# ruc-aimc-lab/LAFF

Hardware: AMD Instinct MI355X
Metric: text-video cosine pairs/sec (higher is better)
Workload: dtype f32 towers (FC on fp16 hi/lo split x3 MFMA) + fp16 similarity

## Files before the change

### laff_amd/csrc/api.hip

```cpp
#include <hip/hip_runtime.h>

#include <algorithm>
#include <climits>
#include <cmath>
#include <cstdarg>
#include <cstdio>
#include <cstdlib>
#include <cstring>
#include <string>
#include <vector>

#include "kernels.h"

constexpr int METRIC_SLOTS = 33;

struct laff_ctx {
    int device;
    hipStream_t stream;
    double* d_metrics = nullptr;
    unsigned metrics_slot = 0;
    double* h_metrics = nullptr;
    char* d_mscratch = nullptr;
};

// ... 1703 lines not shown
    *route = laff::gemm_route(a, sim_gemm_mode(precision), sim_gemm_aligned(K, precision));
    return LAFF_OK;
}

static int rank_prepare_impl(laff_ctx* ctx, const char* who, int sides, int emit, const float* Et, const float* Ev, const void* T,
                             const void* V, int Nt, int Nv, int H, int d, int precision, float prescale, const int* gt_col, int col0,
                             double* s_gt64, float* band_t, float* band_v, int* zero_count, unsigned* pairs) {
    if (int rc = bad_precision(who, precision)) return rc;
    if (Nt < 0 || Nv < 0 || H < 1 || d < 4 || (d & 3)) return fail(LAFF_E_SHAPE, "%s: need H >= 1, d %% 4 == 0 (Nt=%d Nv=%d H=%d d=%d)", who, Nt, Nv, H, d);
    if (!(prescale > 0.0f)) return fail(LAFF_E_ARG, "%s: prescale must be positive", who);
    if ((Et && !aligned16(Et)) || (Ev && !aligned16(Ev)) || (T && !aligned16(T)) || (V && !aligned16(V)))
        return fail(LAFF_E_ALIGN, "%s: embeddings and operands must be 16-byte aligned", who);
    DeviceGuard g(ctx->device);
    HIP_TRY(laff::launch_rank_prepare(Et, Ev, T, V, Nt, Nv, H, d, precision, prescale, gt_col, col0, s_gt64, band_t, band_v, zero_count,
                                      pairs, sides, ctx->stream, emit));
    return LAFF_OK;
}

int laff_rank_prepare(laff_ctx* ctx, const float* Et, const float* Ev, const void* T, const void* V, int Nt, int Nv, int H, int d,
                      int precision, float prescale, const int* gt_col, int col0, double* s_gt64, float* band_t, float* band_v,
                      int* zero_count, unsigned* pairs) {
    CHECK_CTX(ctx);
    if (Nt == 0 && Nv == 0) return LAFF_OK;
    if ((Nt > 0 && (!Et || !T || !gt_col || !s_gt64 || !band_t)) || (Nv > 0 && (!Ev || !V || !band_v)))
        return fail(LAFF_E_ARG, "laff_rank_prepare: null argument");
    return rank_prepare_impl(ctx, "laff_rank_prepare", 3, 0, Et, Ev, T, V, Nt, Nv, H, d, precision, prescale, gt_col, col0, s_gt64, band_t,
                             band_v, zero_count, pairs);
}

int laff_rank_prepare_part(laff_ctx* ctx, int sides, const float* Et, const float* Ev, const void* T, const void* V, int Nt, int Nv, int H,
                           int d, int precision, float prescale, const int* gt_col, int col0, double* s_gt64, float* band_t, float* band_v,
                           int* zero_count, unsigned* pairs) {
    CHECK_CTX(ctx);
    if (sides != 1 && sides != 2) return fail(LAFF_E_ARG, "laff_rank_prepare_part: sides must be 1 (text rows) or 2 (video rows)");
    if ((sides == 1 && Nt == 0) || (sides == 2 && Nv == 0)) return LAFF_OK;
    if (sides == 1 && (!Et || !T || !gt_col || !s_gt64 || !band_t || (Nv > 0 && !Ev))) return fail(LAFF_E_ARG, "laff_rank_prepare_part: null argument (text side)");
    if (sides == 2 && (!Ev || !V || !band_v)) return fail(LAFF_E_ARG, "laff_rank_prepare_part: null argument (video side)");
    return rank_prepare_impl(ctx, "laff_rank_prepare_part", sides, 0, Et, Ev, T, V, Nt, Nv, H, d, precision, prescale, gt_col, col0, s_gt64,
                             band_t, band_v, zero_count, pairs);
}

int laff_rank_prepare_emit(laff_ctx* ctx, int emit, const float* Et, const float* Ev, void* T, void* V, int Nt, int Nv, int H, int d,
                           int precision, float prescale, const int* gt_col, int col0, double* s_gt64, float* band_t, float* band_v,
                           int* zero_count, unsigned* pairs) {
    CHECK_CTX(ctx);
    if (emit < 1 || emit > 3) return fail(LAFF_E_ARG, "laff_rank_prepare_emit: emit must be 1 (T), 2 (V) or 3 (both)");
    if (precision != LAFF_PREC_FP16 && precision != LAFF_PREC_BF16)
        return fail(LAFF_E_UNSUPPORTED, "laff_rank_prepare_emit: single-plane 16-bit operands only (precision %d): call laff_pack_rows + laff_rank_prepare", precision);
    if (Nt == 0 || Nv == 0) return LAFF_OK;
    if (!Et || !Ev || !T || !V || !gt_col || !s_gt64 || !band_t || !band_v) return fail(LAFF_E_ARG, "laff_rank_prepare_emit: null argument");
    return rank_prepare_impl(ctx, "laff_rank_prepare_emit", 3, emit, Et, Ev, T, V, Nt, Nv, H, d, precision, prescale, gt_col, col0, s_gt64,
                             band_t, band_v, zero_count, pairs);
}

int laff_rank_export_pairs(laff_ctx* ctx, const double* s_gt64, int* count, float* S, int lds, int Nv, unsigned* pairs, unsigned pair_cap,
                           const int* bounds, int world, int col0, unsigned* out, unsigned cap, unsigned* fill) {
    CHECK_CTX(ctx);
    if (!s_gt64 || !count || !pairs || !bounds || !out || !fill) return fail(LAFF_E_ARG, "laff_rank_export_pairs: null argument");
    pair_cap &= ~3u;
    if (world < 1 || world > 16 || cap < 4 || (cap & 3) || pair_cap < 4) return fail(LAFF_E_SHAPE, "laff_rank_export_pairs: need 1 <= world <= 16, cap %% 4 == 0 (world=%d cap=%u)", world, cap);
    if (S && lds < Nv) return fail(LAFF_E_SHAPE, "laff_rank_export_pairs: lds=%d < Nv=%d", lds, Nv);
    if (!aligned16(out)) return fail(LAFF_E_ALIGN, "laff_rank_export_pairs: out must be 16-byte aligned");
    DeviceGuard g(ctx->device);
    HIP_TRY(laff::launch_rank_export(s_gt64, count, S, lds, pairs, pair_cap, bounds, world, col0, out, cap, fill, ctx->stream));
    return LAFF_OK;
}

static int rank_resolve_checks(const char* who, const float* Et, const float* Ev, int Nt, int Nv, int H, int d, const double* s_gt64,
                               const int* count, const float* S, int lds, const unsigned* pairs, unsigned& pair_cap) {
    if (!Et || !Ev || !s_gt64 || !count || !pairs) return fail(LAFF_E_ARG, "%s: null argument", who);
    pair_cap &= ~3u;
    if (Nt < 0 || Nv < 0 || H < 1 || d < 4 || (d & 3) || pair_cap < 4) return fail(LAFF_E_SHAPE, "%s: bad shape", who);
    if (S && lds < Nv) return fail(LAFF_E_SHAPE, "%s: lds=%d < Nv=%d", who, lds, Nv);
    if (!aligned16(Et) || !aligned16(Ev)) return fail(LAFF_E_ALIGN, "%s: embeddings must be 16-byte aligned", who);
    return LAFF_OK;
}

int laff_rank_resolve(laff_ctx* ctx, const float* Et, const float* Ev, int Nt, int Nv, int H, int d, const double* s_gt64,
                      int* count, float* S, int lds, unsigned* pairs, unsigned pair_cap) {
    CHECK_CTX(ctx);
    if (Nt == 0 || Nv == 0) return LAFF_OK;
    if (int rc = rank_resolve_checks("laff_rank_resolve", Et, Ev, Nt, Nv, H, d, s_gt64, count, S, lds, pairs, pair_cap)) return rc;
    DeviceGuard g(ctx->device);
    HIP_TRY(laff::launch_rank_resolve(Et, Ev, Nt, Nv, H, d, s_gt64, count, S, lds, pairs, pair_cap, ctx->stream));
    return LAFF_OK;
}

int laff_rank_resolve_metrics(laff_ctx* ctx, const float* Et, const float* Ev, int Nt, int Nv, int H, int d, const double* s_gt64,
                              int* count, float* S, int lds, unsigned* pairs, unsigned pair_cap, int base, int* ranks_out, double* out8,
                              int synchronous) {
    CHECK_CTX(ctx);
    if (!out8) return fail(LAFF_E_ARG, "laff_rank_resolve_metrics: null out8");
    if (Nt < 1 || Nv < 1) return fail(LAFF_E_SHAPE, "laff_rank_resolve_metrics: Nt=%d Nv=%d (the metrics of an empty query set are undefined)", Nt, Nv);
    if (int rc = rank_resolve_checks("laff_rank_resolve_metrics", Et, Ev, Nt, Nv, H, d, s_gt64, count, S, lds, pairs, pair_cap)) return rc;
    DeviceGuard g(ctx->device);
    if (int rc = metrics_buffers(ctx)) return rc;
    const size_t si = synchronous ? 0 : next_metrics_slot(ctx);
    double* slot = ctx->d_metrics + 8 * si;
    unsigned* ticket = (unsigned*)(ctx->d_mscratch + si * laff::rank_metrics_scratch_bytes() + laff::rank_resolve_ticket_offset());
    double* host8 = synchronous ? nullptr : pinned_alias(out8);
    HIP_TRY(laff::launch_rank_resolve(Et, Ev, Nt, Nv, H, d, s_gt64, count, S, lds, pairs, pair_cap, ctx->stream, Nt, base, ranks_out, slot,
                                      host8, ticket));
    if (synchronous) {
        if (int rc = metrics_read_back(ctx, out8, "laff_rank_resolve_metrics: a rank < 1 was found (the pair list of laff_sim_gemm_banded "
                                                  "overflowed, or the counts are corrupt)"))
            return rc;
        out8[7] = 0.0;
        return LAFF_OK;
    }
    if (!host8) HIP_TRY(hipMemcpyAsync(out8, slot, 8 * sizeof(double), hipMemcpyDeviceToHost, ctx->stream));
    return LAFF_OK;
}

int laff_gather_gt(laff_ctx* ctx, const float* S, int Nt, int Nv, int lds, const int* gt_col, int col0, float* s_gt) {
    CHECK_CTX(ctx);
    if (Nt == 0) return LAFF_OK;
    if (!S || !gt_col || !s_gt) return fail(LAFF_E_ARG, "laff_gather_gt: null argument");
    if (Nt < 0 || Nv < 0 || lds < Nv) return fail(LAFF_E_SHAPE, "laff_gather_gt: bad shape");
    DeviceGuard g(ctx->device);
    HIP_TRY(laff::launch_gather_gt(S, Nt, Nv, lds, gt_col, col0, s_gt, ctx->stream));
    return LAFF_OK;
}

int laff_rank_count(laff_ctx* ctx, const float* S, int Nt, int Nv, int lds, const int* gt_col, int col0,
                    const float* s_gt, int* count, int accumulate) {
    CHECK_CTX(ctx);
    if (Nt == 0) return LAFF_OK;
    if (!S || !gt_col || !s_gt || !count) return fail(LAFF_E_ARG, "laff_rank_count: null argument");
    if (Nt < 0 || Nv < 0 || lds < Nv) return fail(LAFF_E_SHAPE, "laff_rank_count: bad shape");
    DeviceGuard g(ctx->device);
    HIP_TRY(laff::launch_rank_count(S, Nt, Nv, lds, gt_col, col0, s_gt, count, accumulate, ctx->stream));
    return LAFF_OK;
}

int laff_topk_rows(laff_ctx* ctx, const float* S, int Nt, int Nv, int lds, int K, int* idx_out, float* val_out) {
    CHECK_CTX(ctx);
    if (Nt == 0) return LAFF_OK;
    if (!S || !idx_out || !val_out) return fail(LAFF_E_ARG, "laff_topk_rows: null argument");
    if (Nt < 0 || Nv < 1 || lds < Nv || K < 1 || K > Nv || K > 8192) return fail(LAFF_E_SHAPE, "laff_topk_rows: need 1 <= K <= min(Nv, 8192) (Nt=%d Nv=%d K=%d)", Nt, Nv, K);
    {
        const size_t kp = K <= 64 ? 64 : (K <= 512 ? 512 : (K <= 2048 ? 2048 : (K <= 4096 ? 4096 : 8192)));
        if ((size_t)((Nv + 3) & ~3) * 4 + kp * 8 + 256 * 4 + 16 > 160 * 1024)
            return fail(LAFF_E_UNSUPPORTED, "laff_topk_rows: Nv=%d with K=%d does not fit the LDS-resident row (%zu columns at most: split the "
                        "columns and merge the per-block lists, as laff_amd.ops.topk_rows does)", Nv, K, (160 * 1024 - kp * 8 - 1040) / 4);
    }
    DeviceGuard g(ctx->device);
    HIP_TRY(laff::launch_topk_rows(S, Nt, Nv, lds, K, idx_out, val_out, ctx->stream));
    return LAFF_OK;
}

int laff_v2t_count(laff_ctx* ctx, const float* S, int Nt, int Nv, int lds, const int* grp_off, const int* grp_idx,
                   int max_group, int* count) {
    CHECK_CTX(ctx);
    if (Nt == 0 || Nv == 0) return LAFF_OK;
    if (!S || !grp_off || !grp_idx || !count) return fail(LAFF_E_ARG, "laff_v2t_count: null argument");
    if (Nt < 0 || Nv < 0 || lds < Nv || max_group < 0) return fail(LAFF_E_SHAPE, "laff_v2t_count: bad shape");
    if (Nt == 0 || Nv == 0 || max_group == 0) return LAFF_OK;
    DeviceGuard g(ctx->device);
    HIP_TRY(laff::launch_v2t_count(S, Nt, Nv, lds, grp_off, grp_idx, max_group, count, ctx->stream));
    return LAFF_OK;
}

int laff_v2t_count_exact(laff_ctx* ctx, const float* S, int Nt, int Nv, int lds, const int* grp_off, const int* grp_idx,
                         int max_group, const float* Et, const float* Ev, int H, int d, const double* s_gt64,
                         const float* band_t, const float* band_v, int* count, unsigned* list, unsigned list_cap) {
    CHECK_CTX(ctx);
    if (Nt == 0 || Nv == 0) return LAFF_OK;
    if (!S || !grp_off || !grp_idx || !count || !Et || !Ev || !s_gt64 || !band_t || !band_v || !list)
        return fail(LAFF_E_ARG, "laff_v2t_count_exact: null argument");
    if (Nt < 0 || Nv < 0 || lds < Nv || max_group < 0 || H < 1 || d < 4 || (d & 3))
        return fail(LAFF_E_SHAPE, "laff_v2t_count_exact: bad shape (Nt=%d Nv=%d lds=%d H=%d d=%d: d must be a multiple of 4)", Nt, Nv, lds, H, d);
    if (!aligned16(Et) || !aligned16(Ev)) return fail(LAFF_E_ALIGN, "laff_v2t_count_exact: embeddings must be 16-byte aligned");
    if (list_cap < 1) return fail(LAFF_E_SHAPE, "laff_v2t_count_exact: list_cap must be >= 1");
    DeviceGuard g(ctx->device);
    if (max_group == 0) {
        HIP_TRY(hipMemsetAsync(count, 0, (size_t)Nt * sizeof(int), ctx->stream));
        HIP_TRY(hipMemsetAsync(list, 0, 16, ctx->stream));
        return LAFF_OK;
    }
    HIP_TRY(laff::launch_v2t_count_exact(S, Nt, Nv, lds, grp_off, grp_idx, max_group, Et, Ev, H, d, s_gt64, band_t, band_v, count, list,
                                         list_cap, ctx->stream));
    return LAFF_OK;
}

int laff_row_dot_gt(laff_ctx* ctx, const void* T, const void* V, int Nt, int Nv, int K, float scale, int precision,
// ... 41 lines not shown
```

### laff_amd/csrc/kernels.h

```cpp
#pragma once
#include <hip/hip_runtime.h>
#include <stdint.h>

#include "../../include/laff_hip.h"

namespace laff {

template <typename K>
static inline hipError_t smem_attr_once(unsigned long long& done, K kernel, int smem) {
    int dev = 0;
    hipError_t e = hipGetDevice(&dev);
    if (e != hipSuccess) return e;
    const unsigned long long bit = 1ull << (dev & 63);
    if (__atomic_load_n(&done, __ATOMIC_ACQUIRE) & bit) return hipSuccess;
    if (smem > 64 * 1024) {
        e = hipFuncSetAttribute((const void*)kernel, hipFuncAttributeMaxDynamicSharedMemorySize, smem);
        if (e != hipSuccess) return e;
    }
    __atomic_fetch_or(&done, bit, __ATOMIC_ACQ_REL);
    return hipSuccess;
}

enum { GEMM_F32 = 0, GEMM_F16 = 1, GEMM_BF16 = 2 };

// ... 147 lines not shown
    const float* g_values[MAX_L];
    const float* g_wt[MAX_L];
    const float* g_bias[MAX_L];
    int g_ldwt[MAX_L], g_dk[MAX_L];
    int head_major;
    int L, N, H, d;
    int head_stride;
    const float* w;
    const float* b;
    const float* gw;
    unsigned flags;
    float* E;
    float* attn_w;
    void* E16;
    int e16_bf16;
    float e16_scale;
    int rp_side;
    const int* rp_gt;
    int rp_col0, rp_Nv;
    const float* rp_Ev;
    double* rp_sgt;
    float* rp_band;
    float* rp_band_v;
    int* rp_count;
    unsigned* rp_pairs;
    double* rp_part;
    unsigned* rp_ticket;
    float rp_unit, rp_cacc;
};
hipError_t launch_fuse(const FuseArgs& a, hipStream_t st);
hipError_t launch_plane_row_norms(const FuseArgs& a, float* out , hipStream_t st);

struct FrameArgs {
    const float* frames;
    const int* lens;
    int B, Fmax, d;
    const float* w;
    const float* b;
    const float* gw;
    unsigned flags;
    float* V;
    const float* mask;
    int ldm;
};
struct FrameGroup {
    int count;
    FrameArgs f[8];
};
hipError_t launch_frame_fuse(const FrameGroup& g, hipStream_t st);

hipError_t launch_split_rows_grouped(int count, const float* const* X, const int* N, const int* K, const int* ldx, void* const* out,
                                     float* const* rscale, hipStream_t st);
hipError_t launch_loss_normalize(const float* s, const float* im, int B, int H, int d, int dp, int Bp, float eps, float* XH,
                                 float* XHT, float* nrm, float* npr, hipStream_t st);
hipError_t launch_margin_reduce(const float* S, float* dS, float* dST, float* loss_h, float* loss, int B, int Bp, int H,
                                float margin, int max_violation, int use_s, int use_im, float g_s, float g_im, hipStream_t st);
hipError_t launch_loss_normalize_bwd(const float* XH, const float* G, const float* nrm, const float* npr, int B, int H, int d,
                                     int dp, float* d_s, float* d_im, hipStream_t st);
hipError_t launch_loss_sum_heads(const float* loss_h, int H, float* loss, hipStream_t st);
constexpr int DSL_STAT_ROWS = 10;
hipError_t launch_dsl_reduce(const float* S, float* ST, float* stat, float* dS, float* dST, float* loss_h, float* loss, int B, int Bp,
                             int H, float temp, hipStream_t st);
hipError_t launch_fc_gather(const int* indptr, const int* indices, const float* values, int N, int Dk, const float* Wt, int ldwt,
                            const float* bias, const float* bn_scale, const float* bn_shift, int D, int act, float* Y, int ldy,
                            hipStream_t st);
hipError_t launch_pack_rows(const float* E, int N, int H, int d, int lde, int normalize, float eps, float prescale,
                            int precision, void* out, hipStream_t st);

hipError_t launch_row_dot_gt(const void* T, const void* V, int Nt, int Nv, int K, int bf16, int x3, float scale,
                             const int* gt_col, int col0, float* s_gt, int* zero_count, hipStream_t st);
static inline void rank_band_constants(int precision, int H, int d, float* unit, float* c_acc) {
    const bool x3 = precision == LAFF_PREC_FP16X3 || precision == LAFF_PREC_BF16X3;
    const bool bf16 = precision == LAFF_PREC_BF16 || precision == LAFF_PREC_BF16X3;
    *unit = precision == LAFF_PREC_FP32 ? 5.9604645e-8f : (bf16 ? 3.90625e-3f : 4.8828125e-4f);
    *c_acc = (float)((double)H * d * (x3 ? 3.0 : 1.0) * 1.1920929e-7 + 9.5367432e-7 + (x3 ? 2.3841858e-7 : 0.0));
}
hipError_t launch_rank_prepare(const float* Et, const float* Ev, const void* T, const void* V, int Nt, int Nv, int H, int d,
                               int precision, float prescale, const int* gt_col, int col0, double* s_gt64, float* band_t,
                               float* band_v, int* zero_count, unsigned* pairs, int sides, hipStream_t st, int emit = 0);
hipError_t launch_rank_export(const double* s_gt64, int* count, float* S, int lds, unsigned* pairs, unsigned pair_cap, const int* bounds,
                              int world, int col0, unsigned* out, unsigned cap, unsigned* fill, hipStream_t st);
hipError_t launch_rank_resolve(const float* Et, const float* Ev, int Nt, int Nv, int H, int d, const double* s_gt64, int* count,
                               float* S, int lds, unsigned* pairs, unsigned pair_cap, hipStream_t st, int metrics_n = 0, int base = 0,
                               int* ranks_out = nullptr, double* out8 = nullptr, double* host8 = nullptr, unsigned* ticket = nullptr);
size_t rank_metrics_scratch_bytes();
size_t rank_resolve_ticket_offset();
hipError_t launch_rank_metrics(const int* r, int n, int base, int* ranks_out, double* out7, double* err, unsigned* scratch, hipStream_t st,
                               double* host8 = nullptr);
hipError_t launch_gather_gt(const float* S, int Nt, int Nv, int lds, const int* gt_col, int col0, float* s_gt,
                            hipStream_t st);
hipError_t launch_rank_count(const float* S, int Nt, int Nv, int lds, const int* gt_col, int col0, const float* s_gt,
                             int* count, int accumulate, hipStream_t st);
hipError_t launch_topk_rows(const float* S, int Nt, int Nv, int lds, int K, int* idx_out, float* val_out, hipStream_t st);
hipError_t launch_v2t_count(const float* S, int Nt, int Nv, int lds, const int* grp_off, const int* grp_idx,
                            int max_group, int* count, hipStream_t st);
hipError_t launch_v2t_count_exact(const float* S, int Nt, int Nv, int lds, const int* grp_off, const int* grp_idx, int max_group,
                                  const float* Et, const float* Ev, int H, int d, const double* s_gt64, const float* band_t,
                                  const float* band_v, int* count, unsigned* list, unsigned cap, hipStream_t st);

struct GruDirArgs {
    const float* P;
    const float* Wp;
    const float* bhh;
    const float* h_in;
    float* h_out;
    float* sum;
    int B;
    int t;
    int col0;
};
struct GruStepArgs {
    GruDirArgs d0, d1;
    const int* tokens;
    const int* lens;
    const int* perm;
    int N, H, V, skip_gemm, pooling;
    float* out;
    int ldo;
};
hipError_t launch_gru_pack_whh(const float* W, int H, float* Wp, hipStream_t st);
hipError_t launch_gru_step(const GruStepArgs& s, int ndirs, hipStream_t st);

typedef float clip_f4 __attribute__((ext_vector_type(4)));
typedef _Float16 clip_h4 __attribute__((ext_vector_type(4)));
typedef _Float16 clip_h8 __attribute__((ext_vector_type(8)));
typedef unsigned clip_u4 __attribute__((ext_vector_type(4)));
#define CLIP_TRY(expr)                               \
    do {                                             \
        const hipError_t e_ = (expr);                \
        if (e_ != hipSuccess) return e_;             \
    } while (0)
enum { CLIP_EPI_F32 = 0, CLIP_EPI_GELU = 1, CLIP_EPI_RESID = 2, CLIP_EPI_GELU_ERF = 3, CLIP_EPI_TANH = 4 };
enum { CLIP_LN_ROW = 0, CLIP_LN_EMBED = 1, CLIP_LN_POOL = 2, CLIP_LN_PATCH = 3 };
struct ClipGemmArgs {
    const void* A;
    const void* B;
    const float* bias;
    void* C;
    int M, N, K, ldc;
};
struct ClipLnArgs {
    float* X;
    const float* gamma;
    const float* beta;
    void* out;
    int W, rows, stride;
    int round_f32;
    const int* ids;
    const int* row_off;
    int N, V, ctx;
    const float* tok_emb;
    const float* pos_emb;
    const float* patch;
    const float* cls;
    const float* pre_gamma;
    const float* pre_beta;
    int L;
};
struct ClipAttnArgs {
    const float* qkv;
    const int* row_off;
    void* out;
    int W;
};
struct ClipEncodeArgs {
    const laff_clip_text* model;
    const int* ids;
    const int* row_off;
    int N, R;
// ... 124 lines not shown
```

### laff_amd/csrc/rank.hip

```cpp
#include <hip/hip_runtime.h>

#include <algorithm>
#include <stdint.h>

#include "kernels.h"
#include "exact_cos.h"
#include "wave_reduce.h"

#ifdef LAFF_TAIL_FENCES
#define LAFF_TICKET_ORDER __ATOMIC_ACQ_REL
#define LAFF_TAIL_RELEASE() __builtin_amdgcn_fence(__ATOMIC_RELEASE, "agent")
#define LAFF_TAIL_ACQUIRE() __builtin_amdgcn_fence(__ATOMIC_ACQUIRE, "agent")
#else
#define LAFF_TICKET_ORDER __ATOMIC_RELAXED
#define LAFF_TAIL_RELEASE() do {} while (0)
#define LAFF_TAIL_ACQUIRE() do {} while (0)
#endif

namespace laff {

__global__ void gather_gt_kernel(const float* __restrict__ S, int Nt, int Nv, long lds, const int* __restrict__ gt_col,
                                 int col0, float* __restrict__ s_gt) {
    const int t = blockIdx.x * blockDim.x + threadIdx.x;
    if (t >= Nt) return;
// ... 508 lines not shown
        if (before <= k && k < before + own) { L.sel[0] = tid; L.sel[1] = before; }
        __syncthreads();
    };
    unsigned prefix = 0, mask = 0;
    int less = 0, shift, below = 0;
    bool below_known = false;
    const int in_lo = (int)L.hist[256];
    if (k < in_lo) {
        select_bin((int)L.hist[tid], 0);
        prefix = (unsigned)L.sel[0]; less = L.sel[1];
        mask = 0xffffffffu;
        shift = -8;
        for (int b = (int)prefix - 1; b >= 1; --b)
            if (L.hist[b]) { below = b; break; }
        below_known = true;
    } else {
        select_bin((int)L.hist[256 + tid], 0);
        const int top = L.sel[0];
        if (top >= 1 && top <= 8) {
            less = L.sel[1];
            select_bin((int)mid[256 * (top - 1) + tid], less);
            prefix = ((unsigned)top << 8) | (unsigned)L.sel[0]; less = L.sel[1];
            mask = 0xffffffffu;
            shift = -8;
        } else if (top < 255) { prefix = (unsigned)top << 8; less = L.sel[1]; mask = 0xffffff00u; shift = 0; }
        else shift = ((32 - __clz(mx | 1) + 7) / 8 - 1) * 8;
    }
    for (; shift >= 0; shift -= 8) {
        __syncthreads();
        for (int i = tid; i < 256 * 9; i += NT) L.hist[i] = 0;
        __syncthreads();
        each([&](int, int vi) {
            const unsigned v = (unsigned)vi;
            if ((v & mask) == prefix) atomicAdd(&L.hist[((v >> shift) & 255u) * 9 + rep8], 1u);
        });
        __syncthreads();
        int own = 0;
#pragma unroll
        for (int q = 0; q < 8; ++q) own += (int)L.hist[tid * 9 + q];
        select_bin(own, less);
        prefix |= (unsigned)L.sel[0] << shift;
        mask |= 255u << shift;
        less = L.sel[1];
    }
    const int med_lo = (int)prefix;
    double med = med_lo;
    if (n > 0 && (n & 1) == 0 && less >= k) {
        if (!below_known) {
            each([&](int, int v) {
                if (v < med_lo) below = max(below, v);
            });
            below = wave_allmax(below);
            __syncthreads();
            if (lane == 0) L.shm[wave][0] = below;
            __syncthreads();
            below = 0;
            for (int w = 0; w < NT / 64; ++w) below = max(below, L.shm[w][0]);
        }
        med = 0.5 * (med + (double)below);
    }
    if (tid == 0) {
        const double dn = (double)n;
        double o[8] = {100.0 * ((double)n1 / dn), 100.0 * ((double)c5 / dn), 100.0 * ((double)c10 / dn), floor(med), (double)sum / dn,
                       isum / dn, isum / dn, 0.0};
#pragma unroll
        for (int i = 0; i < 8; ++i) { out8[i] = o[i]; if (host8) host8[i] = o[i]; }
    }
}

__device__ __forceinline__ void poison_overflow(unsigned* pairs, int* count) {
    __hip_atomic_store(pairs + 1, 1u, __ATOMIC_RELAXED, __HIP_MEMORY_SCOPE_AGENT);
    __hip_atomic_fetch_add(count, -(1 << 26), __ATOMIC_RELAXED, __HIP_MEMORY_SCOPE_AGENT);
}
__device__ __forceinline__ bool list_overflowed(const unsigned* pairs, unsigned pair_cap) {
    if (pairs[2] & 0x80000000u) {
        const unsigned taken = pairs[0], NW = pairs[2] & 0x7fffffffu, NCH = pairs[3];
        return pairs[1] != 0u || NW > NCH || taken > NCH - (NW < NCH ? NW : NCH);
    }
    const unsigned n_over = pairs[0], regA = pairs[2];
    const unsigned long long room = pair_cap > regA ? pair_cap - regA : 0u;
    return pairs[1] != 0u || n_over > room;
}

__device__ __forceinline__ void resolve_groups(const float* __restrict__ Et, const float* __restrict__ Ev, int H, int d,
                                               const double* __restrict__ s_gt64, int* __restrict__ count, float* __restrict__ S,
                                               long lds, unsigned* __restrict__ pairs, unsigned pair_cap,
                                               unsigned (*queue)[RESOLVE_QCAP][2]) {
    const int sl = threadIdx.x & (RG - 1);
    const long K = (long)H * d;
    const unsigned taken = pairs[0], NW = pairs[2] & 0x7fffffffu, NCH = pairs[3];
    const unsigned cnt_words = (NCH + 3u) & ~3u;
    if (pairs[1] != 0u || NW > NCH || taken > NCH - (NW < NCH ? NW : NCH)) {
        if (blockIdx.x == 0 && threadIdx.x == 0) poison_overflow(pairs, count);
    }
    const unsigned long long nchunks = (unsigned long long)NW + taken < NCH ? (unsigned long long)NW + taken : NCH;
    const unsigned long long slots = nchunks * STRIP_CHUNK;
    const unsigned* entries = pairs + 4 + cnt_words;
    (void)pair_cap;
    auto one = [&](unsigned r, unsigned c, bool ok) {
        const double ex = exact_cos(Et + (long)r * K, Ev + (long)c * K, H, d, sl);
        const double sg = s_gt64[r];
        const bool above = ex > sg;
        if (ok && sl == 0) {
            if (above) atomicAdd(count + r, 1);
            if (S) {
                float f = (float)ex;
                const float sgf = (float)sg;
                if (above && !(f > sgf)) f = nextafterf(sgf, INFINITY);
                S[(long)r * lds + c] = f;
            }
        }
    };
    constexpr unsigned QCAP = RESOLVE_QCAP;
    const unsigned wv = threadIdx.x >> 6, sub = (threadIdx.x / RG) & 3u;
    const unsigned group = (blockIdx.x * 256u + threadIdx.x) / RG, ngroups = gridDim.x * (256u / RG);
    unsigned qn = 0;
    auto drain = [&]() {
        for (unsigned i = 0; i < qn; i += 4) {
            const unsigned j = i + sub;
            const bool ok = j < qn;
            const unsigned k = ok ? j : qn - 1;
            one(queue[wv][k][0], queue[wv][k][1], ok);
        }
        qn = 0;
    };
    const unsigned long long trips = (slots + ngroups - 1) / ngroups;
    const unsigned gpb = 256u / RG;
    for (unsigned long long it = 0; it < trips; ++it) {
        if (qn > QCAP - 64) drain();
        const unsigned long long idx = ((unsigned long long)blockIdx.x * trips + it) * gpb + (group % gpb);
        const bool live = idx < slots && (unsigned)(idx % STRIP_CHUNK) < pairs[4 + (unsigned)(idx / STRIP_CHUNK)];
        bool inb = false;
        unsigned row = 0, col = 0;
        if (live) {
            const unsigned* e = entries + idx * STRIP_ENTRY_WORDS;
            const uint4 h0 = *(const uint4*)e;
            const unsigned mask16 = e[4], gt_col = e[5];
            const float x = __uint_as_float(e[8 + sl]);
            const float lo = __uint_as_float(h0.z), hi = __uint_as_float(h0.w);
            row = h0.x;
            col = h0.y + 8u * ((unsigned)sl >> 2) + ((unsigned)sl & 3u);
            if (col == gt_col) {
                if (S) S[(long)row * lds + col] = (float)s_gt64[row];
            } else {
                inb = ((mask16 >> sl) & 1u) && __builtin_amdgcn_fmed3f(x, lo, hi) == x;
            }
        }
        const unsigned long long m = __builtin_amdgcn_ballot_w64(inb);
        if (inb) {
            const unsigned at = qn + __builtin_amdgcn_mbcnt_hi((unsigned)(m >> 32), __builtin_amdgcn_mbcnt_lo((unsigned)m, 0u));
            queue[wv][at][0] = row;
            queue[wv][at][1] = col;
        }
        qn += (unsigned)__builtin_popcountll(m);
    }
    drain();
}

__device__ __forceinline__ void resolve_pairs(const float* __restrict__ Et, const float* __restrict__ Ev, int H, int d,
                                              const double* __restrict__ s_gt64, int* __restrict__ count, float* __restrict__ S,
                                              long lds, unsigned* __restrict__ pairs, unsigned pair_cap,
                                              unsigned (*queue)[RESOLVE_QCAP][2]);

constexpr int RESOLVE_WAVES = 5;
__global__ __launch_bounds__(256) __attribute__((amdgpu_waves_per_eu(RESOLVE_WAVES))) void rank_resolve_kernel(
    const float* __restrict__ Et, const float* __restrict__ Ev, int H, int d, const double* __restrict__ s_gt64, int* __restrict__ count,
    float* __restrict__ S, long lds, unsigned* __restrict__ pairs, unsigned pair_cap, MetricsTail mt) {
    __shared__ __attribute__((aligned(16))) unsigned char pool[RESOLVE_POOL_BYTES];
    unsigned (*queue)[RESOLVE_QCAP][2] = reinterpret_cast<unsigned (*)[RESOLVE_QCAP][2]>(pool);
    const bool overflowed = list_overflowed(pairs, pair_cap);
    if (pairs[2] & 0x80000000u)
        resolve_groups(Et, Ev, H, d, s_gt64, count, S, lds, pairs, pair_cap, queue);
    else
        resolve_pairs(Et, Ev, H, d, s_gt64, count, S, lds, pairs, pair_cap, queue);
    if (mt.n <= 0) return;
    __shared__ unsigned s_ticket;
    asm volatile("s_waitcnt vmcnt(0)" ::: "memory");
    __syncthreads();
    if (threadIdx.x == 0) {
        const unsigned g = blockIdx.x % RESOLVE_TICKET_GROUPS, gsz = (gridDim.x - g + RESOLVE_TICKET_GROUPS - 1u) / RESOLVE_TICKET_GROUPS;
        const unsigned ngroups = gridDim.x < RESOLVE_TICKET_GROUPS ? gridDim.x : RESOLVE_TICKET_GROUPS;
        unsigned* const tg = mt.ticket + 64u * (1u + g);
        unsigned last = 0u;
        LAFF_TAIL_RELEASE();
        if (__hip_atomic_fetch_add(tg, 1u, LAFF_TICKET_ORDER, __HIP_MEMORY_SCOPE_AGENT) == gsz - 1u) {
            __hip_atomic_store(tg, 0u, __ATOMIC_RELAXED, __HIP_MEMORY_SCOPE_AGENT);
            if (__hip_atomic_fetch_add(mt.ticket, 1u, LAFF_TICKET_ORDER, __HIP_MEMORY_SCOPE_AGENT) == ngroups - 1u) {
                __hip_atomic_store(mt.ticket, 0u, __ATOMIC_RELAXED, __HIP_MEMORY_SCOPE_AGENT);
                last = 1u;
            }
        }
        s_ticket = last;
    }
    __syncthreads();
    if (!s_ticket) return;
    __builtin_amdgcn_fence(__ATOMIC_ACQUIRE, "agent");
    metrics_single_block<256>(count, mt.n, mt.base, mt.ranks_out, mt.out8, mt.host8, *reinterpret_cast<MetricsLds*>(pool), overflowed);
}

__device__ __forceinline__ void resolve_pairs(const float* __restrict__ Et, const float* __restrict__ Ev, int H, int d,
                                              const double* __restrict__ s_gt64, int* __restrict__ count, float* __restrict__ S,
                                              long lds, unsigned* __restrict__ pairs, unsigned pair_cap,
                                              unsigned (*queue)[RESOLVE_QCAP][2]) {
    const int sl = threadIdx.x & (RG - 1);
    const long K = (long)H * d;
    constexpr unsigned QCAP = RESOLVE_QCAP;
    const unsigned n_over = pairs[0], regA = pairs[2];
    const unsigned long long room = pair_cap > regA ? pair_cap - regA : 0u;
    if (n_over > room) {
        if (blockIdx.x == 0 && threadIdx.x == 0) poison_overflow(pairs, count);
    }
    auto one = [&](unsigned r, unsigned c, bool ok) {
        const double ex = exact_cos(Et + (long)r * K, Ev + (long)c * K, H, d, sl);
        const double sg = s_gt64[r];
        const bool above = ex > sg;
        if (ok && sl == 0) {
            if (above) atomicAdd(count + r, 1);
            if (S) {
                float f = (float)ex;
                const float sgf = (float)sg;
                if (above && !(f > sgf)) f = nextafterf(sgf, INFINITY);
                S[(long)r * lds + c] = f;
            }
        }
    };
    const unsigned wv = threadIdx.x >> 6, sub = (threadIdx.x / RG) & 3u, lane = threadIdx.x & 63u;
    const unsigned n = (unsigned)(n_over < room ? n_over : room);
    const unsigned long long total = (unsigned long long)regA + n;
    const unsigned group = (blockIdx.x * 256u + threadIdx.x) / RG, ngroups = gridDim.x * (256u / RG);
    unsigned qn = 0;
    auto drain = [&]() {
        for (unsigned i = 0; i < qn; i += 4) {
            const unsigned j = i + sub;
            const bool ok = j < qn;
            const unsigned k = ok ? j : qn - 1;
            one(queue[wv][k][0], queue[wv][k][1], ok);
        }
        qn = 0;
    };
    const unsigned long long trips = (total + 4ull * ngroups - 1) / (4ull * ngroups);
    for (unsigned long long it = 0; it < trips; ++it) {
        if (qn > QCAP - 16) drain();
        const unsigned long long s0 = 4ull * (it * ngroups + group);
        uint4 p0 = make_uint4(0xffffffffu, 0, 0xffffffffu, 0), p1 = p0;
        if (s0 < total) {
            p0 = *(const uint4*)(pairs + 4 + 2 * s0);
            if (p0.x != 0xffffffffu && s0 + 2 < total) p1 = *(const uint4*)(pairs + 4 + 2 * s0 + 4);
        }
        const unsigned rs[4] = {p0.x, p0.z, p1.x, p1.z}, cs[4] = {p0.y, p0.w, p1.y, p1.w};
#pragma unroll
        for (int k = 0; k < 4; ++k) {
            const bool v = sl == 0 && s0 + k < total && rs[k] != 0xffffffffu;
            const unsigned long long m = __builtin_amdgcn_ballot_w64(v);
            if (v) {
// ... 60 lines not shown
            }
        }
        qn = 0;
    };
    auto push = [&](bool v, unsigned row, unsigned col) {
        const unsigned long long m = __builtin_amdgcn_ballot_w64(v);
        if (v) {
            const unsigned at = qn + __builtin_amdgcn_mbcnt_hi((unsigned)(m >> 32), __builtin_amdgcn_mbcnt_lo((unsigned)m, 0u));
            queue[wv][at][0] = row;
            queue[wv][at][1] = col;
            queue[wv][at][2] = owner(row);
        }
        qn += (unsigned)__builtin_popcountll(m);
    };
    const unsigned group = (blockIdx.x * 256u + threadIdx.x) / RG, ngroups = gridDim.x * (256u / RG);
    if (pairs[2] & 0x80000000u) {
        const unsigned taken = pairs[0], NW = pairs[2] & 0x7fffffffu, NCH = pairs[3];
        const unsigned cnt_words = (NCH + 3u) & ~3u;
        if ((pairs[1] != 0u || NW > NCH || taken > NCH - (NW < NCH ? NW : NCH)) && blockIdx.x == 0 && threadIdx.x == 0) poison();
        const unsigned long long nchunks = (unsigned long long)NW + taken < NCH ? (unsigned long long)NW + taken : NCH;
        const unsigned long long slots = nchunks * STRIP_CHUNK;
        const unsigned* entries = pairs + 4 + cnt_words;
        const unsigned long long trips = (slots + ngroups - 1) / ngroups;
        for (unsigned long long it = 0; it < trips; ++it) {
            if (qn > EXPORT_QCAP - 64) drain();
            const unsigned long long idx = it * ngroups + group;
            const bool live = idx < slots && (unsigned)(idx % STRIP_CHUNK) < pairs[4 + (unsigned)(idx / STRIP_CHUNK)];
            bool inb = false;
            unsigned row = 0, col = 0;
            if (live) {
                const unsigned* e = entries + idx * STRIP_ENTRY_WORDS;
                const uint4 h0 = *(const uint4*)e;
                const unsigned mask16 = e[4], gt_col = e[5];
                const float v = __uint_as_float(e[8 + sl]);
                const float lo = __uint_as_float(h0.z), hi = __uint_as_float(h0.w);
                row = h0.x;
                col = h0.y + 8u * ((unsigned)sl >> 2) + ((unsigned)sl & 3u);
                if (col == gt_col) {
                    if (S) S[(long)row * lds + col] = (float)s_gt64[row];
                } else {
                    inb = ((mask16 >> sl) & 1u) && __builtin_amdgcn_fmed3f(v, lo, hi) == v;
                }
            }
            push(inb, row, col);
        }
    } else {
        const unsigned n_over = pairs[0], regA = pairs[2];
        const unsigned long long room = pair_cap > regA ? pair_cap - regA : 0u;
        if (n_over > room && blockIdx.x == 0 && threadIdx.x == 0) poison();
        const unsigned n = (unsigned)(n_over < room ? n_over : room);
        const unsigned long long total = (unsigned long long)regA + n;
        const unsigned long long nthreads = (unsigned long long)gridDim.x * 256u;
        const unsigned long long trips = (total + nthreads - 1) / nthreads;
        for (unsigned long long it = 0; it < trips; ++it) {
            if (qn > EXPORT_QCAP - 64) drain();
            const unsigned long long i = it * nthreads + (unsigned long long)blockIdx.x * 256u + threadIdx.x;
            unsigned row = 0xffffffffu, col = 0;
            if (i < total) { row = pairs[4 + 2 * i]; col = pairs[4 + 2 * i + 1]; }
            push(row != 0xffffffffu, row, col);
        }
    }
    drain();
}

__global__ __launch_bounds__(256) void rank_export_init_kernel(uint4* __restrict__ out, size_t n16, unsigned* __restrict__ fill, int world) {
    const size_t i0 = (size_t)blockIdx.x * 256 + threadIdx.x, step = (size_t)gridDim.x * 256;
    for (size_t i = i0; i < n16; i += step) out[i] = make_uint4(0xffffffffu, 0xffffffffu, 0xffffffffu, 0xffffffffu);
    if (i0 <= (size_t)world) fill[i0] = 0u;
}

hipError_t launch_rank_export(const double* s_gt64, int* count, float* S, int lds, unsigned* pairs, unsigned pair_cap, const int* bounds,
                              int world, int col0, unsigned* out, unsigned cap, unsigned* fill, hipStream_t st) {
    if (world < 1 || world > 16 || (cap & 3)) return hipErrorInvalidValue;
    const size_t n16 = (size_t)world * cap / 2;
    hipLaunchKernelGGL(rank_export_init_kernel, dim3((unsigned)std::min<size_t>((n16 + 255) / 256, (size_t)(8 * g_num_cus))), dim3(256), 0, st,
                       (uint4*)out, n16, fill, world);
    ExportArgs x{bounds, world, col0, out, cap, fill};
    hipLaunchKernelGGL(rank_export_kernel, dim3((unsigned)(4 * g_num_cus)), dim3(256), 0, st, s_gt64, count, S, (long)lds, pairs, pair_cap, x);
    return hipGetLastError();
}

hipError_t launch_rank_resolve(const float* Et, const float* Ev, int Nt, int Nv, int H, int d, const double* s_gt64, int* count,
                               float* S, int lds, unsigned* pairs, unsigned pair_cap, hipStream_t st, int metrics_n, int base,
                               int* ranks_out, double* out8, double* host8, unsigned* ticket) {
    (void)Nt; (void)Nv;
    MetricsTail mt{metrics_n, base, ranks_out, out8, host8, ticket};
    hipLaunchKernelGGL(rank_resolve_kernel, dim3((unsigned)(RESOLVE_WAVES * g_num_cus)), dim3(256), 0, st, Et, Ev, H, d, s_gt64, count, S, (long)lds, pairs,
                       pair_cap, mt);
    return hipGetLastError();
}

constexpr int MS_GMAX = 256;
struct MetricsPartial { unsigned long long c1, c5, c10, sum; double isum; int mx, mn; int pad[4]; };
static_assert(sizeof(MetricsPartial) == 64, "scratch layout");
constexpr size_t MS_BYTES = 4096 + (size_t)MS_GMAX * sizeof(MetricsPartial);
size_t rank_metrics_scratch_bytes() { return MS_BYTES + ((RESOLVE_TICKET_BYTES + 4095) & ~(size_t)4095); }
size_t rank_resolve_ticket_offset() { return MS_BYTES; }

__global__ __launch_bounds__(1024) void rank_metrics_kernel(const int* __restrict__ r, int n, int base, int* __restrict__ ranks_out,
                                                            double* __restrict__ out7, double* __restrict__ err,
                                                            unsigned* __restrict__ scratch, double* __restrict__ host8) {
    __shared__ double shd[16];
    __shared__ unsigned long long shl[16][4];
    __shared__ int shm[16][2];
    __shared__ unsigned hist[256 * 33];
    __shared__ int wsum[4];
    __shared__ int sel[2];
    __shared__ unsigned s_ticket;
    const int tid = threadIdx.x, lane = tid & 63, wave = tid >> 6;
    const int G = (int)gridDim.x;
    unsigned* const ghist = scratch + 4;
    MetricsPartial* const parts = (MetricsPartial*)((char*)scratch + 4096);

    for (int i = tid; i < 512 * 9; i += 1024) hist[i] = 0;
    __syncthreads();
    unsigned long long c1 = 0, c5 = 0, c10 = 0, sum = 0;
    double isum = 0;
    int mx = 0, mn = 0x7fffffff;
    const int rep8 = lane & 7;
    for (long i = (long)blockIdx.x * 1024 + tid; i < n; i += (long)G * 1024) {
        const int v = r[i] + base;
        if (ranks_out) ranks_out[i] = v;
        c1 += v <= 1; c5 += v <= 5; c10 += v <= 10;
        sum += (unsigned long long)(long long)v;
        const double d = (double)v;
        double q = (double)__builtin_amdgcn_rcpf((float)v);
        q = q * (2.0 - d * q);
        q = q * (2.0 - d * q);
        isum += q;
        mx = max(mx, v); mn = min(mn, v);
        const unsigned u = (unsigned)v;
        if (u < 256u) atomicAdd(&hist[u * 9 + rep8], 1u);
        atomicAdd(&hist[(256u + min(u >> 8, 255u)) * 9 + rep8], 1u);
    }
    auto block_sums = [&]() {
        c1 = wave_allsum(c1); c5 = wave_allsum(c5); c10 = wave_allsum(c10); sum = wave_allsum(sum);
        isum = wave_allsum(isum);
        mx = wave_allmax(mx); mn = wave_allmin(mn);
        if (lane == 0) {
            shl[wave][0] = c1; shl[wave][1] = c5; shl[wave][2] = c10; shl[wave][3] = sum;
            shd[wave] = isum;
            shm[wave][0] = mx; shm[wave][1] = mn;
        }
        __syncthreads();
        if (tid == 0) {
            c1 = c5 = c10 = sum = 0; isum = 0; mx = 0; mn = 0x7fffffff;
            for (int w = 0; w < 16; ++w) {
                c1 += shl[w][0]; c5 += shl[w][1]; c10 += shl[w][2]; sum += shl[w][3]; isum += shd[w];
                mx = max(mx, shm[w][0]); mn = min(mn, shm[w][1]);
            }
        }
    };
    block_sums();
    if (tid == 0) {
        unsigned long long* q = (unsigned long long*)(parts + blockIdx.x);
        const unsigned long long w[6] = {c1, c5, c10, sum, (unsigned long long)__double_as_longlong(isum),
                                         (unsigned long long)(unsigned)mx | ((unsigned long long)(unsigned)mn << 32)};
#pragma unroll
        for (int k = 0; k < 6; ++k) __hip_atomic_store(q + k, w[k], __ATOMIC_RELAXED, __HIP_MEMORY_SCOPE_AGENT);
    }
    if (tid < 512) {
        unsigned t = 0;
#pragma unroll
        for (int q = 0; q < 8; ++q) t += hist[tid * 9 + q];
        if (t) __hip_atomic_fetch_add(ghist + tid, t, __ATOMIC_RELAXED, __HIP_MEMORY_SCOPE_AGENT);
    }
    asm volatile("s_waitcnt vmcnt(0)" ::: "memory");
    __syncthreads();
    if (tid == 0) {
        LAFF_TAIL_RELEASE();
        s_ticket = __hip_atomic_fetch_add(scratch, 1u, LAFF_TICKET_ORDER, __HIP_MEMORY_SCOPE_AGENT);
    }
    __syncthreads();
    if (s_ticket != (unsigned)(G - 1)) return;
    LAFF_TAIL_ACQUIRE();

    {
        c1 = c5 = c10 = sum = 0; isum = 0; mx = 0; mn = 0x7fffffff;
        if (tid < G) {
            const unsigned long long* q = (const unsigned long long*)(parts + tid);
// ... 385 lines not shown
```

Baseline: 428.0 billion.

## Bin resolve pairs by video column bucket before exact-cosine resolution

Adds a binning kernel that sorts the banded candidate pairs into a fixed number of buckets by video column, placed in the unused tail of the pair buffer. The resolve kernel then has blocks assigned per bucket, so each block recomputes exact cosines over a narrow range of video embeddings, which is meant to improve cache reuse of Ev rows. Bucket counters are reset through a ticket scheme. In exchange it adds an extra kernel launch, global atomics and spare-buffer requirements, and falls back to the old path when the buckets overflow.

Result: slower. 421.7 billion (-1.5%).

```diff
diff --git a/laff_amd/csrc/api.hip b/laff_amd/csrc/api.hip
--- a/laff_amd/csrc/api.hip
+++ b/laff_amd/csrc/api.hip
@@ -1809,7 +1809,10 @@
     if (Nt == 0 || Nv == 0) return LAFF_OK;
     if (int rc = rank_resolve_checks("laff_rank_resolve", Et, Ev, Nt, Nv, H, d, s_gt64, count, S, lds, pairs, pair_cap)) return rc;
     DeviceGuard g(ctx->device);
-    HIP_TRY(laff::launch_rank_resolve(Et, Ev, Nt, Nv, H, d, s_gt64, count, S, lds, pairs, pair_cap, ctx->stream));
+    if (int rc = metrics_buffers(ctx)) return rc;
+    char* scratch = ctx->d_mscratch + next_metrics_slot(ctx) * laff::rank_metrics_scratch_bytes();
+    HIP_TRY(laff::launch_rank_resolve(Et, Ev, Nt, Nv, H, d, s_gt64, count, S, lds, pairs, pair_cap, ctx->stream, 0, 0, nullptr, nullptr, nullptr,
+                                      nullptr, (unsigned*)(scratch + laff::rank_resolve_bucket_offset())));
     return LAFF_OK;
 }
 
@@ -1824,10 +1827,11 @@
     if (int rc = metrics_buffers(ctx)) return rc;
     const size_t si = synchronous ? 0 : next_metrics_slot(ctx);
     double* slot = ctx->d_metrics + 8 * si;
-    unsigned* ticket = (unsigned*)(ctx->d_mscratch + si * laff::rank_metrics_scratch_bytes() + laff::rank_resolve_ticket_offset());
+    char* scratch = ctx->d_mscratch + si * laff::rank_metrics_scratch_bytes();
+    unsigned* ticket = (unsigned*)(scratch + laff::rank_resolve_ticket_offset());
     double* host8 = synchronous ? nullptr : pinned_alias(out8);
     HIP_TRY(laff::launch_rank_resolve(Et, Ev, Nt, Nv, H, d, s_gt64, count, S, lds, pairs, pair_cap, ctx->stream, Nt, base, ranks_out, slot,
-                                      host8, ticket));
+                                      host8, ticket, (unsigned*)(scratch + laff::rank_resolve_bucket_offset())));
     if (synchronous) {
         if (int rc = metrics_read_back(ctx, out8, "laff_rank_resolve_metrics: a rank < 1 was found (the pair list of laff_sim_gemm_banded "
                                                   "overflowed, or the counts are corrupt)"))
diff --git a/laff_amd/csrc/kernels.h b/laff_amd/csrc/kernels.h
--- a/laff_amd/csrc/kernels.h
+++ b/laff_amd/csrc/kernels.h
@@ -253,9 +253,11 @@
                               int world, int col0, unsigned* out, unsigned cap, unsigned* fill, hipStream_t st);
 hipError_t launch_rank_resolve(const float* Et, const float* Ev, int Nt, int Nv, int H, int d, const double* s_gt64, int* count,
                                float* S, int lds, unsigned* pairs, unsigned pair_cap, hipStream_t st, int metrics_n = 0, int base = 0,
-                               int* ranks_out = nullptr, double* out8 = nullptr, double* host8 = nullptr, unsigned* ticket = nullptr);
+                               int* ranks_out = nullptr, double* out8 = nullptr, double* host8 = nullptr, unsigned* ticket = nullptr,
+                               unsigned* bucket_ctr = nullptr);
 size_t rank_metrics_scratch_bytes();
 size_t rank_resolve_ticket_offset();
+size_t rank_resolve_bucket_offset();
 hipError_t launch_rank_metrics(const int* r, int n, int base, int* ranks_out, double* out7, double* err, unsigned* scratch, hipStream_t st,
                                double* host8 = nullptr);
 hipError_t launch_gather_gt(const float* S, int Nt, int Nv, int lds, const int* gt_col, int col0, float* s_gt,
diff --git a/laff_amd/csrc/rank.hip b/laff_amd/csrc/rank.hip
--- a/laff_amd/csrc/rank.hip
+++ b/laff_amd/csrc/rank.hip
@@ -614,6 +614,129 @@
     return pairs[1] != 0u || n_over > room;
 }
 
+constexpr unsigned RESOLVE_BUCKETS = 8;
+constexpr unsigned BUCKET_CTR_STRIDE = 64;
+constexpr unsigned BUCKET_TICKET0 = RESOLVE_BUCKETS * BUCKET_CTR_STRIDE;
+struct BucketView { unsigned* rec; unsigned cap; };
+__device__ __forceinline__ BucketView bucket_view(unsigned* pairs, unsigned pair_cap) {
+    unsigned long long used;
+    if (pairs[2] & 0x80000000u) {
+        const unsigned taken = pairs[0], NW = pairs[2] & 0x7fffffffu, NCH = pairs[3];
+        const unsigned long long nchunks = (unsigned long long)NW + taken < NCH ? (unsigned long long)NW + taken : NCH;
+        used = 4ull + ((NCH + 3u) & ~3u) + nchunks * STRIP_CHUNK * STRIP_ENTRY_WORDS;
+    } else {
+        const unsigned n_over = pairs[0], regA = pairs[2];
+        const unsigned long long room = pair_cap > regA ? pair_cap - regA : 0u;
+        used = 4ull + 2ull * ((unsigned long long)regA + (n_over < room ? n_over : room));
+    }
+    used = (used + 3ull) & ~3ull;
+    const unsigned long long total = 4ull + 2ull * pair_cap;
+    const unsigned long long cap = total > used ? (total - used) / (2ull * RESOLVE_BUCKETS) : 0ull;
+    return BucketView{pairs + used, (unsigned)(cap < 0x7fffffffull ? cap : 0x7fffffffull)};
+}
+__device__ __forceinline__ unsigned bucket_of(unsigned col, int Nv) {
+    const unsigned long long x = (unsigned long long)col * RESOLVE_BUCKETS / (unsigned)(Nv > 0 ? Nv : 1);
+    return (unsigned)(x < RESOLVE_BUCKETS ? x : RESOLVE_BUCKETS - 1);
+}
+
+constexpr unsigned BIN_QCAP = 2048;
+__global__ __launch_bounds__(256) void rank_bin_kernel(const double* __restrict__ s_gt64, float* __restrict__ S, long lds,
+                                                       unsigned* __restrict__ pairs, unsigned pair_cap, int Nv, unsigned* __restrict__ ctr) {
+    __shared__ unsigned queue[BIN_QCAP][2];
+    __shared__ unsigned s_qn, s_cnt[RESOLVE_BUCKETS], s_base[RESOLVE_BUCKETS];
+    if (list_overflowed(pairs, pair_cap)) return;
+    const BucketView bv = bucket_view(pairs, pair_cap);
+    const unsigned tid = threadIdx.x, lane = tid & 63u;
+    const int sl = threadIdx.x & (RG - 1);
+    if (tid == 0) s_qn = 0u;
+    if (tid < RESOLVE_BUCKETS) s_cnt[tid] = 0u;
+    __syncthreads();
+    auto push = [&](bool v, unsigned row, unsigned col) {
+        const unsigned long long m = __builtin_amdgcn_ballot_w64(v);
+        if (m == 0ull) return;
+        unsigned base = 0;
+        if (lane == 0) base = atomicAdd(&s_qn, (unsigned)__builtin_popcountll(m));
+        base = __builtin_amdgcn_readfirstlane(base);
+        if (v) {
+            const unsigned at = base + __builtin_amdgcn_mbcnt_hi((unsigned)(m >> 32), __builtin_amdgcn_mbcnt_lo((unsigned)m, 0u));
+            queue[at][0] = row;
+            queue[at][1] = col;
+        }
+    };
+    auto flush = [&]() {
+        const unsigned qn = s_qn;
+        for (unsigned i = tid; i < qn; i += 256u) atomicAdd(&s_cnt[bucket_of(queue[i][1], Nv)], 1u);
+        __syncthreads();
+        if (tid < RESOLVE_BUCKETS) {
+            const unsigned c = s_cnt[tid];
+            s_base[tid] = c ? __hip_atomic_fetch_add(ctr + tid * BUCKET_CTR_STRIDE, c, __ATOMIC_RELAXED, __HIP_MEMORY_SCOPE_AGENT) : 0u;
+            s_cnt[tid] = 0u;
+        }
+        __syncthreads();
+        for (unsigned i = tid; i < qn; i += 256u) {
+            const unsigned row = queue[i][0], col = queue[i][1], o = bucket_of(col, Nv);
+            const unsigned pos = s_base[o] + atomicAdd(&s_cnt[o], 1u);
+            if (pos < bv.cap)
+                *(uint2*)(bv.rec + 2ull * ((unsigned long long)o * bv.cap + pos)) = make_uint2(row, col);
+        }
+        __syncthreads();
+        if (tid == 0) s_qn = 0u;
+        if (tid < RESOLVE_BUCKETS) s_cnt[tid] = 0u;
+        __syncthreads();
+    };
+    auto flush_if_full = [&]() {
+        __syncthreads();
+        const bool full = s_qn > BIN_QCAP - 256u;
+        __syncthreads();
+        if (full) flush();
+    };
+    if (pairs[2] & 0x80000000u) {
+        const unsigned taken = pairs[0], NW = pairs[2] & 0x7fffffffu, NCH = pairs[3];
+        const unsigned cnt_words = (NCH + 3u) & ~3u;
+        const unsigned long long nchunks = (unsigned long long)NW + taken < NCH ? (unsigned long long)NW + taken : NCH;
+        const unsigned long long slots = nchunks * STRIP_CHUNK;
+        const unsigned* entries = pairs + 4 + cnt_words;
+        const unsigned gpb = 256u / RG, ngroups = gridDim.x * gpb;
+        const unsigned long long trips = (slots + ngroups - 1) / ngroups;
+        for (unsigned long long it = 0; it < trips; ++it) {
+            flush_if_full();
+            const unsigned long long idx = ((unsigned long long)blockIdx.x * trips + it) * gpb + tid / RG;
+            const bool live = idx < slots && (unsigned)(idx % STRIP_CHUNK) < pairs[4 + (unsigned)(idx / STRIP_CHUNK)];
+            bool inb = false;
+            unsigned row = 0, col = 0;
+            if (live) {
+                const unsigned* e = entries + idx * STRIP_ENTRY_WORDS;
+                const uint4 h0 = *(const uint4*)e;
+                const unsigned mask16 = e[4], gt_col = e[5];
+                const float x = __uint_as_float(e[8 + sl]);
+                const float lo = __uint_as_float(h0.z), hi = __uint_as_float(h0.w);
+                row = h0.x;
+                col = h0.y + 8u * ((unsigned)sl >> 2) + ((unsigned)sl & 3u);
+                if (col == gt_col) {
+                    if (S) S[(long)row * lds + col] = (float)s_gt64[row];
+                } else {
+                    inb = ((mask16 >> sl) & 1u) && __builtin_amdgcn_fmed3f(x, lo, hi) == x;
+                }
+            }
+            push(inb, row, col);
+        }
+    } else {
+        const unsigned n_over = pairs[0], regA = pairs[2];
+        const unsigned long long room = pair_cap > regA ? pair_cap - regA : 0u;
+        const unsigned long long total = (unsigned long long)regA + (n_over < room ? n_over : room);
+        const unsigned long long trips = (total + (unsigned long long)gridDim.x * 256u - 1) / ((unsigned long long)gridDim.x * 256u);
+        for (unsigned long long it = 0; it < trips; ++it) {
+            flush_if_full();
+            const unsigned long long i = ((unsigned long long)blockIdx.x * trips + it) * 256u + tid;
+            unsigned row = 0xffffffffu, col = 0;
+            if (i < total) { const uint2 p = *(const uint2*)(pairs + 4 + 2 * i); row = p.x; col = p.y; }
+            push(row != 0xffffffffu, row, col);
+        }
+    }
+    __syncthreads();
+    flush();
+}
+
 __device__ __forceinline__ void resolve_groups(const float* __restrict__ Et, const float* __restrict__ Ev, int H, int d,
                                                const double* __restrict__ s_gt64, int* __restrict__ count, float* __restrict__ S,
                                                long lds, unsigned* __restrict__ pairs, unsigned pair_cap,
@@ -694,14 +817,81 @@
                                               long lds, unsigned* __restrict__ pairs, unsigned pair_cap,
                                               unsigned (*queue)[RESOLVE_QCAP][2]);
 
+__device__ __forceinline__ void resolve_bucket(const float* __restrict__ Et, const float* __restrict__ Ev, int H, int d,
+                                               const double* __restrict__ s_gt64, int* __restrict__ count, float* __restrict__ S,
+                                               long lds, const unsigned* __restrict__ rec, unsigned n) {
+    const int sl = threadIdx.x & (RG - 1);
+    const long K = (long)H * d;
+    const unsigned wv = threadIdx.x >> 6, sub = (threadIdx.x / RG) & 3u;
+    const unsigned j = blockIdx.x / RESOLVE_BUCKETS;
+    const unsigned nj = (gridDim.x - blockIdx.x % RESOLVE_BUCKETS + RESOLVE_BUCKETS - 1u) / RESOLVE_BUCKETS;
+    const unsigned long long per = (((unsigned long long)n + nj - 1u) / nj + 15ull) & ~15ull;
+    const unsigned long long s0 = (unsigned long long)j * per;
+    const unsigned long long end = s0 + per < n ? s0 + per : n;
+    for (unsigned long long i = s0 + 4u * wv; i < end; i += 16u) {
+        const bool ok = i + sub < end;
+        const uint2 p = *(const uint2*)(rec + 2ull * (ok ? i + sub : end - 1u));
+        const unsigned r = p.x, c = p.y;
+        const double ex = exact_cos(Et + (long)r * K, Ev + (long)c * K, H, d, sl);
+        const double sg = s_gt64[r];
+        const bool above = ex > sg;
+        if (ok && sl == 0) {
+            if (above) atomicAdd(count + r, 1);
+            if (S) {
+                float f = (float)ex;
+                const float sgf = (float)sg;
+                if (above && !(f > sgf)) f = nextafterf(sgf, INFINITY);
+                S[(long)r * lds + c] = f;
+            }
+        }
+    }
+}
+
 constexpr int RESOLVE_WAVES = 5;
 __global__ __launch_bounds__(256) __attribute__((amdgpu_waves_per_eu(RESOLVE_WAVES))) void rank_resolve_kernel(
     const float* __restrict__ Et, const float* __restrict__ Ev, int H, int d, const double* __restrict__ s_gt64, int* __restrict__ count,
-    float* __restrict__ S, long lds, unsigned* __restrict__ pairs, unsigned pair_cap, MetricsTail mt) {
+    float* __restrict__ S, long lds, unsigned* __restrict__ pairs, unsigned pair_cap, MetricsTail mt, unsigned* __restrict__ bctr) {
     __shared__ __attribute__((aligned(16))) unsigned char pool[RESOLVE_POOL_BYTES];
     unsigned (*queue)[RESOLVE_QCAP][2] = reinterpret_cast<unsigned (*)[RESOLVE_QCAP][2]>(pool);
+    __shared__ unsigned s_bucket[2];
     const bool overflowed = list_overflowed(pairs, pair_cap);
-    if (pairs[2] & 0x80000000u)
+    bool bucketed = false;
+    if (bctr && !overflowed) {
+        const BucketView bv = bucket_view(pairs, pair_cap);
+        if (threadIdx.x == 0) {
+            unsigned fits = 1u, mine = 0u;
+#pragma unroll
+            for (unsigned o = 0; o < RESOLVE_BUCKETS; ++o) {
+                const unsigned f = __hip_atomic_load(bctr + o * BUCKET_CTR_STRIDE, __ATOMIC_RELAXED, __HIP_MEMORY_SCOPE_AGENT);
+                if (f > bv.cap) fits = 0u;
+                if (o == blockIdx.x % RESOLVE_BUCKETS) mine = f;
+            }
+            s_bucket[0] = fits; s_bucket[1] = mine;
+        }
+        __syncthreads();
+        bucketed = s_bucket[0] != 0u;
+        if (threadIdx.x == 0) {
+            const unsigned g = blockIdx.x % RESOLVE_TICKET_GROUPS, gsz = (gridDim.x - g + RESOLVE_TICKET_GROUPS - 1u) / RESOLVE_TICKET_GROUPS;
+            const unsigned ngroups = gridDim.x < RESOLVE_TICKET_GROUPS ? gridDim.x : RESOLVE_TICKET_GROUPS;
+            unsigned* const top = bctr + BUCKET_TICKET0;
+            unsigned* const tg = top + BUCKET_CTR_STRIDE * (1u + g);
+            asm volatile("s_waitcnt vmcnt(0)" ::: "memory");
+            if (__hip_atomic_fetch_add(tg, 1u, __ATOMIC_RELAXED, __HIP_MEMORY_SCOPE_AGENT) == gsz - 1u) {
+                __hip_atomic_store(tg, 0u, __ATOMIC_RELAXED, __HIP_MEMORY_SCOPE_AGENT);
+                if (__hip_atomic_fetch_add(top, 1u, __ATOMIC_RELAXED, __HIP_MEMORY_SCOPE_AGENT) == ngroups - 1u) {
+                    __hip_atomic_store(top, 0u, __ATOMIC_RELAXED, __HIP_MEMORY_SCOPE_AGENT);
+#pragma unroll
+                    for (unsigned o = 0; o < RESOLVE_BUCKETS; ++o)
+                        __hip_atomic_store(bctr + o * BUCKET_CTR_STRIDE, 0u, __ATOMIC_RELAXED, __HIP_MEMORY_SCOPE_AGENT);
+                }
+            }
+        }
+        if (bucketed)
+            resolve_bucket(Et, Ev, H, d, s_gt64, count, S, lds,
+                           bv.rec + 2ull * (unsigned long long)(blockIdx.x % RESOLVE_BUCKETS) * bv.cap, s_bucket[1]);
+    }
+    if (bucketed) {}
+    else if (pairs[2] & 0x80000000u)
         resolve_groups(Et, Ev, H, d, s_gt64, count, S, lds, pairs, pair_cap, queue);
     else
         resolve_pairs(Et, Ev, H, d, s_gt64, count, S, lds, pairs, pair_cap, queue);
@@ -928,11 +1118,12 @@
 
 hipError_t launch_rank_resolve(const float* Et, const float* Ev, int Nt, int Nv, int H, int d, const double* s_gt64, int* count,
                                float* S, int lds, unsigned* pairs, unsigned pair_cap, hipStream_t st, int metrics_n, int base,
-                               int* ranks_out, double* out8, double* host8, unsigned* ticket) {
-    (void)Nt; (void)Nv;
+                               int* ranks_out, double* out8, double* host8, unsigned* ticket, unsigned* bctr) {
+    (void)Nt;
+    if (bctr) hipLaunchKernelGGL(rank_bin_kernel, dim3((unsigned)g_num_cus), dim3(256), 0, st, s_gt64, S, (long)lds, pairs, pair_cap, Nv, bctr);
     MetricsTail mt{metrics_n, base, ranks_out, out8, host8, ticket};
     hipLaunchKernelGGL(rank_resolve_kernel, dim3((unsigned)(RESOLVE_WAVES * g_num_cus)), dim3(256), 0, st, Et, Ev, H, d, s_gt64, count, S, (long)lds, pairs,
-                       pair_cap, mt);
+                       pair_cap, mt, bctr);
     return hipGetLastError();
 }
 
@@ -940,8 +1131,10 @@
 struct MetricsPartial { unsigned long long c1, c5, c10, sum; double isum; int mx, mn; int pad[4]; };
 static_assert(sizeof(MetricsPartial) == 64, "scratch layout");
 constexpr size_t MS_BYTES = 4096 + (size_t)MS_GMAX * sizeof(MetricsPartial);
-size_t rank_metrics_scratch_bytes() { return MS_BYTES + ((RESOLVE_TICKET_BYTES + 4095) & ~(size_t)4095); }
+constexpr size_t RESOLVE_BUCKET_CTR_BYTES = 256 * (RESOLVE_BUCKETS + 1 + RESOLVE_TICKET_GROUPS);
+size_t rank_metrics_scratch_bytes() { return MS_BYTES + ((RESOLVE_TICKET_BYTES + RESOLVE_BUCKET_CTR_BYTES + 4095) & ~(size_t)4095); }
 size_t rank_resolve_ticket_offset() { return MS_BYTES; }
+size_t rank_resolve_bucket_offset() { return MS_BYTES + RESOLVE_TICKET_BYTES; }
 
 __global__ __launch_bounds__(1024) void rank_metrics_kernel(const int* __restrict__ r, int n, int base, int* __restrict__ ranks_out,
                                                             double* __restrict__ out7, double* __restrict__ err,
```
